# ghazalehnt/RecBole

Measured on AMD Instinct MI355X. Metric: train positives/sec (+neg) per node, higher is better.
Workload: dtype fp32; 1 GPU; C2 BPR-MF ml-20m-shape: 138,494 users x 26,745 items (incl. PAD), ~20M interactions RO_RS 0.8/0.1/0.1, embedding 128, 4 uniform negatives, 512 positives (2,048 rows) per step, dense Adam; global_batch=512, per_gpu_batch=512, train_interactions=16014928, parallelism=single, exchange_graph=True, sampler=walk (bit-exact)

## Files before the change

recbole_amd/csrc/adam.hip:

```cpp

#include "adam_core.h"

namespace mirec {

template <int D>
__global__ __launch_bounds__(kAdamThreads) void adam_multi_kernel(
    const AdamTables tabs, const float* __restrict__ consts, const int32_t* __restrict__ step_base,
    int step_off, AdamConsts k) {
  constexpr int VPR = D / 4;
  constexpr int RPP = kAdamThreads / VPR;
  static_assert(kAdamThreads % VPR == 0, "row width");
  __shared__ int32_t slot[kAdamRows];
  __shared__ int32_t s_range[2];

  const int si = segment_of(tabs, blockIdx.x);
  const mirec_adam_table& T = tabs.t[si];
  float* __restrict__ P = T.p;
  float* __restrict__ M = T.m;
  float* __restrict__ V = T.v;
  const int32_t* __restrict__ uniq = T.uniq;

  const int64_t lo = ((int64_t)blockIdx.x - tabs.block_start[si]) * kAdamRows;
  const int64_t hi = min(T.n_rows, lo + kAdamRows);
  if (threadIdx.x < kAdamRows) slot[threadIdx.x] = -1;
// ... 125 lines not shown
    const int i = base + rsub;
    const bool work = i < n;
    const int64_t r = lo + (work ? s_row[i] : 0);
    const int last = work ? min(s_last[i], target) : target;
    const int64_t off = r * VPR + c;
    V p, m, v;
    memset(&p, 0, sizeof(V));
    m = p;
    v = p;
    if (work) {
      p = reinterpret_cast<const V*>(T.p)[off];
      m = reinterpret_cast<const V*>(T.m)[off];
      v = reinterpret_cast<const V*>(T.v)[off];
    }
    adam_replay(p, m, v, last, target, consts, k);
    if (work) {
      reinterpret_cast<V*>(T.p)[off] = p;
      reinterpret_cast<V*>(T.m)[off] = m;
      reinterpret_cast<V*>(T.v)[off] = v;
      if (c == 0) T.last[r] = target;
    }
  }
}

template <int D>
struct FlushVec { using T = float; };
template <> struct FlushVec<128> { using T = float2; };
template <> struct FlushVec<256> { using T = float4; };

#ifndef MIREC_FLUSH_THREADS
#define MIREC_FLUSH_THREADS 64
#endif
constexpr int kFlushRowThreads = MIREC_FLUSH_THREADS;

template <int D>
__device__ __forceinline__ void flush_row(const mirec_adam_table& T, int64_t r, int raw,
                                          int target, int lane,
                                          const float* __restrict__ consts,
                                          const AdamConsts& k) {
  using V = typename FlushVec<D>::T;
  const int last = min(raw, target);
  const int64_t off = r * 64 + lane;
  const bool par = T.p_alt != nullptr;
  const bool odd = par && (target & 1);
  if (last >= target) {
    if (odd && raw != kZeroState)
      reinterpret_cast<V*>(T.p)[off] = reinterpret_cast<const V*>(T.p_alt)[off];
    return;
  }
  V p = reinterpret_cast<const V*>((par && (last & 1)) ? T.p_alt : T.p)[off];
  V m = reinterpret_cast<const V*>(T.m)[off];
  V v = reinterpret_cast<const V*>(T.v)[off];
  replay<V, true>(p, m, v, last, target, consts, k);
  MIREC_WORK(10, 1);
  if (odd) reinterpret_cast<V*>(T.p_alt)[off] = p;
  reinterpret_cast<V*>(T.p)[off] = p;
  reinterpret_cast<V*>(T.m)[off] = m;
  reinterpret_cast<V*>(T.v)[off] = v;
  if (lane == 0) T.last[r] = target;
}

__device__ __forceinline__ bool flush_needs(const mirec_adam_table& T, int raw, int target) {
  return min(raw, target) < target || (T.p_alt != nullptr && (target & 1) && raw != kZeroState);
}

template <int D>
__global__ __launch_bounds__(kFlushRowThreads) void adam_flush_row_kernel(
    const AdamTables tabs, const float* __restrict__ consts, const int32_t* __restrict__ step_base,
    int step_off, AdamConsts k) {
  constexpr int RPB = kFlushRowThreads / 64;
  const int si = segment_of(tabs, blockIdx.x);
  const mirec_adam_table& T = tabs.t[si];
  const int64_t r = ((int64_t)blockIdx.x - tabs.block_start[si]) * RPB + (threadIdx.x >> 6);
  if (r >= T.n_rows) return;
  const int target = step_base[0] + step_off;
  const int raw = __builtin_amdgcn_readfirstlane(T.last[r]);
  flush_row<D>(T, r, raw, target, threadIdx.x & 63, consts, k);
}

constexpr int64_t kScanOneWaveMax = 1 << 17;
struct FlushRows {
  int32_t r[kMaxTables];
};
struct FlushMasks {
  const uint32_t* bits[kMaxTables];
  int32_t want[kMaxTables];
};

__device__ __forceinline__ bool mask_selects(const uint32_t* __restrict__ bits, int want,
                                             int64_t r) {
  return !bits || (int)((bits[r >> 5] >> (r & 31)) & 1u) == want;
}

template <int D, bool MASKED>
__global__ __launch_bounds__(kAdamThreads) void adam_flush_scan_kernel(
    const AdamTables tabs, const float* __restrict__ consts, const int32_t* __restrict__ step_base,
    int step_off, AdamConsts k, FlushRows rows_per_wave, FlushMasks masks) {
  const int si = segment_of(tabs, blockIdx.x);
  const mirec_adam_table& T = tabs.t[si];
  const int R = rows_per_wave.r[si];
  const int lane = threadIdx.x & 63;
  const int64_t r0 =
      (((int64_t)blockIdx.x - tabs.block_start[si]) * (blockDim.x >> 6) + (threadIdx.x >> 6)) * R;
  if (r0 >= T.n_rows) return;
  const int target = step_base[0] + step_off;
  int raw = kZeroState;
  if (lane < R && r0 + lane < T.n_rows &&
      (!MASKED || mask_selects(masks.bits[si], masks.want[si], r0 + lane)))
    raw = T.last[r0 + lane];
  uint64_t todo = __ballot(flush_needs(T, raw, target));
  while (todo) {
    const int i = __builtin_ctzll(todo);
    todo &= todo - 1;
    flush_row<D>(T, r0 + i, __shfl(raw, i, 64), target, lane, consts, k);
  }
}

struct FlushFirst {
  const int32_t* first[kMaxTables];
};
constexpr int kFirstNotRead = MIREC_FIRST_NOT_READ;

template <int D>
__global__ __launch_bounds__(kAdamThreads) void adam_flush_first_kernel(
    const AdamTables tabs, const float* __restrict__ consts, const int32_t* __restrict__ step_base,
    int step_off, AdamConsts k, FlushRows rows_per_wave, FlushFirst ff) {
  const int si = segment_of(tabs, blockIdx.x);
  const mirec_adam_table& T = tabs.t[si];
  const int R = rows_per_wave.r[si];
  const int lane = threadIdx.x & 63;
  const int64_t r0 =
      (((int64_t)blockIdx.x - tabs.block_start[si]) * (blockDim.x >> 6) + (threadIdx.x >> 6)) * R;
  if (r0 >= T.n_rows) return;
  const int base = step_base[0] + step_off;
  int raw = kZeroState, target = 0;
  if (lane < R && r0 + lane < T.n_rows) {
    const int f = ff.first[si][r0 + lane];
    if (f > kFirstNotRead) {
      target = base + f;
      raw = T.last[r0 + lane];
    }
  }
  uint64_t todo = __ballot(min(raw, target) < target);
  while (todo) {
    const int i = __builtin_ctzll(todo);
    todo &= todo - 1;
    flush_row<D>(T, r0 + i, __builtin_amdgcn_readfirstlane(__shfl(raw, i, 64)),
                 __builtin_amdgcn_readfirstlane(__shfl(target, i, 64)), lane, consts, k);
  }
}

constexpr int kWalkRows = 32;

template <int D>
__global__ __launch_bounds__(64) void adam_flush_walk_kernel(
    const AdamTables tabs, const float* __restrict__ consts, const int32_t* __restrict__ step_base,
    int step_off, AdamConsts k, FlushMasks masks) {
  const int lane = threadIdx.x;
  const int target = step_base[0] + step_off;
  for (int si = 0; si < tabs.n_seg; ++si) {
    const mirec_adam_table& T = tabs.t[si];
    const uint32_t* __restrict__ bits = masks.bits[si];
    const uint32_t flip = masks.want[si] ? 0u : ~0u;
    const int64_t groups = (T.n_rows + kWalkRows - 1) / kWalkRows;
    for (int64_t g = blockIdx.x; g < groups; g += gridDim.x) {
      const int64_t r0 = g * kWalkRows;
      const uint32_t sel = bits ? (bits[g] ^ flip) : ~0u;
      int raw = kZeroState;
      if (lane < kWalkRows && r0 + lane < T.n_rows && ((sel >> lane) & 1u))
        raw = T.last[r0 + lane];
      uint64_t todo = __ballot(flush_needs(T, raw, target));
      while (todo) {
        const int i = __builtin_ctzll(todo);
        todo &= todo - 1;
        flush_row<D>(T, r0 + i, __shfl(raw, i, 64), target, lane, consts, k);
      }
    }
  }
}

}

using namespace mirec;

namespace {

enum class Sched { kStreamed, kDeferred, kFlush, kDeferredPair };

int launch_adam(Sched sched, const mirec_adam_table* tables, int32_t n_tables,
                const int64_t* n_max_uniq, int32_t d, const float* consts,
                const int32_t* step_base, int32_t step_off, double beta1, double beta2,
                double eps, double weight_decay, void* stream, const char* what,
                const int32_t* flush_rows = nullptr, const FlushMasks* masks = nullptr,
                int walk_waves = 0, const FlushFirst* firsts = nullptr) {
  if (n_tables < 1 || n_tables > kMaxTables || !tables || !consts || !step_base) {
    set_error("%s: bad arguments (n_tables=%d)", what, n_tables);
    return -1;
  }
  if (((uintptr_t)consts & 15) != 0) {
    set_error("%s: step constants must be 16-byte aligned", what);
    return -1;
  }
  if (d != 4 && d != 16 && d != 32 && d != 64 && d != 128 && d != 256 &&
      !(d == 1 && sched != Sched::kStreamed)) {
    set_error("%s: row width %d not in {4,16,32,64,128,256} (1: deferred / flush)", what, d);
    return -1;
  }
  const int VPR = d / 4;
  const bool pair = sched == Sched::kDeferredPair;
  if (pair) {
    if (n_tables != 2 || d == 1) {
      set_error("%s: a pair is two tables, the first of width d > 1 (got %d tables, d=%d)",
                what, n_tables, d);
      return -1;
    }
    sched = Sched::kDeferred;
  }
  FlushRows fr;
  bool scan = false;
  for (int q = 0; q < kMaxTables; ++q) fr.r[q] = 1;
  if (sched == Sched::kFlush && flush_rows) {
    if (d < 64) {
      set_error("%s: rows per wave need d >= 64", what);
      return -1;
    }
    for (int q = 0; q < n_tables; ++q) {
      if (flush_rows[q] < 1 || flush_rows[q] > 64) {
        set_error("%s: rows per wave %d of table %d not in [1, 64]", what, flush_rows[q], q);
        return -1;
      }
      fr.r[q] = flush_rows[q];
    }
    scan = true;
  }
  const bool walk = masks && walk_waves > 0;
  if (masks && (sched != Sched::kFlush || d < 64 || (!scan && !walk))) {
    set_error("%s: a masked flush needs d >= 64 and rows per wave or a wave count", what);
    return -1;
  }
  FlushMasks fm;
  memset(&fm, 0, sizeof(fm));
  if (masks) fm = *masks;
  if (firsts && (sched != Sched::kFlush || !scan || masks)) {
    set_error("%s: per-row targets need the flush with rows per wave and no mask", what);
    return -1;
  }
  FlushFirst ff;
  memset(&ff, 0, sizeof(ff));
  if (firsts) ff = *firsts;
  int scan_threads = kAdamThreads;
  if (scan && !walk) {
    int64_t waves = 0;
    for (int q = 0; q < n_tables; ++q)
      if (tables[q].n_rows > 0) waves += (tables[q].n_rows + fr.r[q] - 1) / fr.r[q];
    if (waves <= kScanOneWaveMax) scan_threads = 64;
  }
  AdamTables tabs;
  memset(&tabs, 0, sizeof(tabs));
  const bool deferred = sched == Sched::kDeferred;
  tabs.n_seg = deferred ? 2 * n_tables : n_tables;
  int dvec = 1;
  if (deferred && n_max_uniq && d >= 4) {
    int64_t waves = 0;
    for (int q = 0; q < (pair ? 1 : n_tables); ++q)
      if (n_max_uniq[q] > 0)
        waves += n_max_uniq[q] * (tables[q].ahead_uniq ? 2 : 1) * ((d + 63) / 64);
    if (waves > 16 * 1024) dvec = 2;
    bool ahead = false;
    for (int q = 0; q < n_tables; ++q) ahead = ahead || tables[q].ahead_uniq != nullptr;
    if (dvec == 2 && d >= 128 && !ahead && !pair) dvec = 4;
  }
  int64_t blocks = 0;
  for (int q = 0; q < n_tables; ++q) {
    const mirec_adam_table& t = tables[q];
    const bool grouped = t.n_uniq != nullptr;
    if (!t.p || !t.m || !t.v || t.n_rows < 0 ||
        (grouped && (!t.uniq || !t.seg || !t.perm || !t.rows)) ||
        (sched != Sched::kStreamed && !t.last) ||
        (deferred && (!grouped || t.dense_grad || !n_max_uniq || n_max_uniq[q] < 0)) ||
        (deferred && (t.ahead_uniq == nullptr) != (t.ahead_n_uniq == nullptr))) {
      set_error("%s: bad table %d", what, q);
      return -1;
    }
    if (t.p_alt && (sched == Sched::kStreamed || d < 64 || pair)) {
      set_error("%s: table %d: parity buffer (p_alt) needs the deferred schedule and d >= 64",
                what, q);
      return -1;
    }
    tabs.t[q] = t;
    if (walk) {
      tabs.block_start[q] = 0;
      if (t.n_rows > 0) blocks = walk_waves;
    } else if (deferred) {
      const int rpb = (pair && q == 1) ? deferred_block(1) : deferred_block(d / dvec) / (d / dvec);
      const int64_t nb = (n_max_uniq[q] + rpb - 1) / rpb;
      tabs.block_start[2 * q] = blocks;
      blocks += nb;
      tabs.block_start[2 * q + 1] = blocks;
      if (t.ahead_uniq) blocks += nb;
    } else {
      tabs.block_start[q] = blocks;
      const int64_t rows_per_block =
          scan ? (int64_t)(scan_threads / 64) * fr.r[q]
          : (sched == Sched::kFlush && d >= 64) ? kFlushRowThreads / 64
          : sched == Sched::kFlush ? kFlushRows
                                   : kAdamRows;
      blocks += (t.n_rows + rows_per_block - 1) / rows_per_block;
    }
  }
  (void)VPR;
  for (int q = tabs.n_seg; q <= 2 * kMaxTables; ++q) tabs.block_start[q] = blocks;
  if (blocks == 0) return 0;
  AdamConsts k;
  k.omb1 = (float)(1.0 - beta1);
  k.omb1m1 = k.omb1 - 1.0f;
  k.lerp_small = fabsf(k.omb1) < 0.5f;
  k.b2 = (float)beta2;
  k.omb2 = (float)(1.0 - beta2);
  k.eps = (float)eps;
  k.wd = (float)weight_decay;
  const dim3 grd((unsigned)blocks), blk(kAdamThreads);
  hipStream_t st = (hipStream_t)stream;
#define MIREC_ADAM_SCHED(DD)                                                                 \
  case DD:                                                                                   \
    if (sched == Sched::kStreamed)                                                           \
      hipLaunchKernelGGL(adam_multi_kernel<DD>, grd, blk, 0, st, tabs, consts, step_base,    \
                         step_off, k);                                                       \
    else if (deferred && pair)                                                               \
      hipLaunchKernelGGL((dvec == 2 ? adam_deferred_pair_kernel<DD, float2>                  \
                                    : adam_deferred_pair_kernel<DD, float>),                 \
                         grd, dim3(deferred_block(1)), 0, st, tabs, consts, step_base,       \
                         step_off, k);                                                       \
    else if (deferred)                                                                       \
      hipLaunchKernelGGL((dvec == 4 ? adam_deferred_kernel<DD, float4>                       \
                          : dvec == 2 ? adam_deferred_kernel<DD, float2>                     \
                                      : adam_deferred_kernel<DD, float>),                    \
                         grd, dim3(deferred_block(DD / dvec)), 0, st, tabs, consts,          \
                         step_base, step_off, k);                                            \
    else if (DD >= 64 && walk)                                                               \
      hipLaunchKernelGGL(adam_flush_walk_kernel<(DD >= 64 ? DD : 64)>, grd, dim3(64), 0, st,   \
                         tabs, consts, step_base, step_off, k, fm);                          \
    else if (DD >= 64 && scan && firsts)                                                     \
      hipLaunchKernelGGL(adam_flush_first_kernel<(DD >= 64 ? DD : 64)>, grd,                 \
                         dim3(scan_threads), 0, st, tabs, consts, step_base, step_off, k,    \
                         fr, ff);                                                            \
    else if (DD >= 64 && scan && masks)                                                      \
      hipLaunchKernelGGL((adam_flush_scan_kernel<(DD >= 64 ? DD : 64), true>), grd,          \
                         dim3(scan_threads), 0, st, tabs, consts, step_base, step_off, k,    \
                         fr, fm);                                                            \
    else if (DD >= 64 && scan)                                                               \
      hipLaunchKernelGGL((adam_flush_scan_kernel<(DD >= 64 ? DD : 64), false>), grd,         \
                         dim3(scan_threads), 0, st, tabs, consts, step_base, step_off, k,    \
                         fr, fm);                                                            \
    else if (DD >= 64)                                                                       \
      hipLaunchKernelGGL(adam_flush_row_kernel<(DD >= 64 ? DD : 64)>, grd,                   \
                         dim3(kFlushRowThreads), 0, st, tabs,                                \
                         consts, step_base, step_off, k);                                    \
    else                                                                                     \
      hipLaunchKernelGGL(adam_flush_list_kernel<(DD < 64 ? DD : 16)>, grd, blk, 0, st, tabs, \
                         consts, step_base, step_off, k);                                    \
    break;
  switch (d) {
    case 1:
      if (deferred)
        hipLaunchKernelGGL((adam_deferred_kernel<1, float>), grd, dim3(deferred_block(1)), 0, st,
                           tabs, consts, step_base, step_off, k);
      else
        hipLaunchKernelGGL(adam_flush_list_kernel<1>, grd, blk, 0, st, tabs, consts, step_base,
                           step_off, k);
      break;
    MIREC_ADAM_SCHED(4)
    MIREC_ADAM_SCHED(16)
    MIREC_ADAM_SCHED(32)
    MIREC_ADAM_SCHED(64)
    MIREC_ADAM_SCHED(128)
    MIREC_ADAM_SCHED(256)
  }
#undef MIREC_ADAM_SCHED
  return launch_status(what);
}

}

extern "C" int mirec_adam_multi_f32(const mirec_adam_table* tables, int32_t n_tables, int32_t d,
                                    const float* step_consts_dev, const int32_t* step_base_dev,
                                    int32_t step_off, double beta1, double beta2, double eps,
                                    double weight_decay, void* stream) {
  return launch_adam(Sched::kStreamed, tables, n_tables, nullptr, d, step_consts_dev,
                     step_base_dev, step_off, beta1, beta2, eps, weight_decay, stream,
                     "mirec_adam_multi_f32");
}

extern "C" int mirec_adam_deferred_f32(const mirec_adam_table* tables, int32_t n_tables,
                                       const int64_t* n_max_uniq, int32_t d,
                                       const float* step_consts_dev,
                                       const int32_t* step_base_dev, int32_t step_off,
                                       double beta1, double beta2, double eps,
                                       double weight_decay, void* stream) {
  return launch_adam(Sched::kDeferred, tables, n_tables, n_max_uniq, d, step_consts_dev,
                     step_base_dev, step_off, beta1, beta2, eps, weight_decay, stream,
                     "mirec_adam_deferred_f32");
}

extern "C" int mirec_adam_deferred_pair_f32(const mirec_adam_table* tables,
                                            const int64_t* n_max_uniq, int32_t d,
                                            const float* step_consts_dev,
                                            const int32_t* step_base_dev, int32_t step_off,
                                            double beta1, double beta2, double eps,
                                            double weight_decay, void* stream) {
  return launch_adam(Sched::kDeferredPair, tables, 2, n_max_uniq, d, step_consts_dev,
                     step_base_dev, step_off, beta1, beta2, eps, weight_decay, stream,
                     "mirec_adam_deferred_pair_f32");
}

extern "C" int mirec_adam_flush_f32(const mirec_adam_table* tables, int32_t n_tables, int32_t d,
                                    const float* step_consts_dev, const int32_t* step_base_dev,
                                    int32_t step_off, double beta1, double beta2, double eps,
                                    double weight_decay, void* stream) {
  return launch_adam(Sched::kFlush, tables, n_tables, nullptr, d, step_consts_dev,
                     step_base_dev, step_off, beta1, beta2, eps, weight_decay, stream,
                     "mirec_adam_flush_f32");
}

#if defined(MIREC_STEP_COUNT)
extern "C" int mirec_work_counters_adam(unsigned long long* dst, int clear) {
  if (hipMemcpyFromSymbol(dst, HIP_SYMBOL(g_work), sizeof(g_work)) != hipSuccess) return -1;
  if (clear) {
    unsigned long long z[16] = {0};
    if (hipMemcpyToSymbol(HIP_SYMBOL(g_work), z, sizeof(z)) != hipSuccess) return -1;
  }
  return 0;
}
#endif

extern "C" int mirec_adam_flush_rows_f32(const mirec_adam_table* tables, int32_t n_tables,
                                         int32_t d, const int32_t* rows_per_wave,
                                         const float* step_consts_dev,
                                         const int32_t* step_base_dev, int32_t step_off,
                                         double beta1, double beta2, double eps,
                                         double weight_decay, void* stream) {
  if (!rows_per_wave) {
    set_error("mirec_adam_flush_rows_f32: rows_per_wave is NULL");
    return -1;
  }
  return launch_adam(Sched::kFlush, tables, n_tables, nullptr, d, step_consts_dev,
                     step_base_dev, step_off, beta1, beta2, eps, weight_decay, stream,
                     "mirec_adam_flush_rows_f32", rows_per_wave);
}

extern "C" int mirec_adam_flush_masked_f32(const mirec_adam_table* tables, int32_t n_tables,
                                           int32_t d, const uint32_t* const* masks,
                                           const int32_t* want, const int32_t* rows_per_wave,
                                           int32_t walk_waves, const float* step_consts_dev,
                                           const int32_t* step_base_dev, int32_t step_off,
                                           double beta1, double beta2, double eps,
                                           double weight_decay, void* stream) {
  const char* what = "mirec_adam_flush_masked_f32";
  if (!tables || n_tables < 1 || n_tables > kMaxTables || !want || walk_waves < 0 ||
      walk_waves > 65536 || (walk_waves == 0) != (rows_per_wave != nullptr)) {
    set_error("%s: bad arguments (rows per wave for the scan form, or a wave count in "
              "[1, 65536] for the walk form)", what);
    return -1;
  }
  mirec_adam_table sel[kMaxTables];
  int32_t rows[kMaxTables];
  FlushMasks fm;
  memset(&fm, 0, sizeof(fm));
  int n = 0;
  for (int q = 0; q < n_tables; ++q) {
    if (want[q] < 0) continue;
    if (want[q] > 1) {
      set_error("%s: want[%d] = %d not in {-1, 0, 1}", what, q, want[q]);
      return -1;
    }
    sel[n] = tables[q];
    rows[n] = rows_per_wave ? rows_per_wave[q] : 1;
    fm.bits[n] = masks ? masks[q] : nullptr;
    fm.want[n] = want[q];
    ++n;
  }
  if (n == 0) return 0;
  return launch_adam(Sched::kFlush, sel, n, nullptr, d, step_consts_dev, step_base_dev, step_off,
                     beta1, beta2, eps, weight_decay, stream, what,
                     rows_per_wave ? rows : nullptr, &fm, walk_waves);
}

extern "C" int mirec_adam_flush_first_f32(const mirec_adam_table* tables, int32_t n_tables,
                                          int32_t d, const int32_t* const* first,
                                          const int32_t* rows_per_wave,
                                          const float* step_consts_dev,
                                          const int32_t* step_base_dev, int32_t step_off,
                                          double beta1, double beta2, double eps,
                                          double weight_decay, void* stream) {
  const char* what = "mirec_adam_flush_first_f32";
// ... 188 lines not shown
```

recbole_amd/csrc/step.hip:

```cpp
#include "adam_core.h"
#include "bpr_math.h"
#include "ahead.h"

namespace mirec {

struct StepLaunch {
  mirec_adam_table t[2];
  const int32_t* rec[2];
  const int32_t* crec[2];
  float* part[2];
  int32_t* join[2];
  int64_t block_start[7];
  int32_t seg_rows[6];
};

__device__ __forceinline__ int64_t clamp_id(int64_t id, int64_t n) {
  return id < 0 ? 0 : (id >= n ? n - 1 : id);
}


constexpr int kRecInts = 8;
constexpr int kRecInline = 2;
constexpr int kRowRec = 4 + kRecInline * kRecInts;
constexpr int kShare = kRecInline;
// ... 219 lines not shown
      run += c[j];
    }
  }
  __syncthreads();
#pragma unroll
  for (int r = 0; r < kGrpEpt; ++r) {
    const int e = tid + r * kGrpThreads;
    if (e < per) L.xb[L.bstart[keys[e] >> shift] + slot_in[r]] = x[r];
  }
  __syncthreads();
#pragma unroll
  for (int r = 0; r < kGrpEpt; ++r) {
    const int e = tid + r * kGrpThreads;
    if (e < per) {
      const int bk = keys[e] >> shift;
      const int b0 = L.bstart[bk], n = L.hist[bk];
      int rank = 0;
      for (int f = 0; f < n; ++f) rank += L.xb[b0 + f] < x[r] ? 1 : 0;
      L.xa[b0 + rank] = x[r];
    }
  }
  __syncthreads();
  const uint32_t* S = L.xa;
  int32_t* __restrict__ perm = J.perm + (int64_t)b * per;
  int32_t* __restrict__ uniq = J.uniq + (int64_t)b * per;
  int32_t* __restrict__ seg = J.seg + (int64_t)b * (per + 1);
  int hm = 0, cnt = 0;
#pragma unroll
  for (int r = 0; r < kGrpEpt; ++r) {
    const int e = kGrpEpt * tid + r;
    if (e < per) {
      const uint32_t k = S[e] >> pbits;
      const int h = (e == 0 || (S[e - 1] >> pbits) != k) ? 1 : 0;
      hm |= h << r;
      cnt += h;
      perm[e] = (int32_t)(S[e] & ((1u << pbits) - 1u));
    }
  }
  int nu;
  int slot = block_exclusive_scan(cnt, L.scan, &nu);
#pragma unroll
  for (int r = 0; r < kGrpEpt; ++r) {
    if ((hm >> r) & 1) {
      const int e = kGrpEpt * tid + r;
      const int32_t k = (int32_t)(S[e] >> pbits);
      L.srow[slot] = k;
      L.sseg[slot] = e;
      uniq[slot] = k;
      seg[slot] = e;
      ++slot;
    }
  }
  if (tid == 0) {
    L.sseg[nu] = per;
    seg[nu] = per;
    J.nu[b] = nu;
  }
  __syncthreads();
  if (J.rec != nullptr) {
    int32_t* __restrict__ rec = J.rec + (int64_t)b * rec_ints(per);
    int32_t* __restrict__ task = rec + (int64_t)per * kRowRec;
    const uint32_t pm = (1u << pbits) - 1u;
    int dealt = 0;
    for (int x0 = 0; x0 < nu; x0 += kGrpThreads) {
      const int xs = x0 + tid;
      int i0 = 0, nc = 0, row = 0;
      if (xs < nu) {
        i0 = L.sseg[xs];
        nc = L.sseg[xs + 1] - i0;
        row = L.srow[xs];
      }
      const int want = nc > kShare ? (nc + kShare - 1) / kShare - 1 : 0;
      int total;
      const int base = dealt + block_exclusive_scan(want, L.scan, &total);
      dealt += total;
      if (xs >= nu) continue;
      const int got = max(0, min(want, kSplitCap - base));
      const int nsh = 1 + got;
      int32_t* r = rec + (int64_t)xs * kRowRec;
      reinterpret_cast<int4*>(r)[0] = make_int4(row, i0, nc, nsh);
      for (int c = 0; c < kRecInline && c < nc; ++c)
        contrib_record_lds((int)(S[i0 + c] & pm), tb, Bc, T, L.uk, L.ik, r + 4 + c * kRecInts);
      for (int jj = 1; jj <= got; ++jj) {
        int32_t* tr = task + (int64_t)(base + jj - 1) * kTaskRec;
        reinterpret_cast<int4*>(tr)[0] = make_int4(xs, jj, i0, nc);
        reinterpret_cast<int4*>(tr)[1] = make_int4(row, nsh, 0, 0);
        for (int c = 0; c < kShare && jj * kShare + c < nc; ++c)
          contrib_record_lds((int)(S[i0 + jj * kShare + c] & pm), tb, Bc, T, L.uk, L.ik,
                             tr + 8 + c * kRecInts);
      }
    }
    if (tid == 0) task[(int64_t)kSplitCap * kTaskRec] = min(dealt, kSplitCap);
    int32_t* __restrict__ crec = J.crec + (int64_t)b * per * kRecInts;
    for (int e = tid; e < per; e += kGrpThreads)
      contrib_record_lds((int)(S[e] & pm), tb, Bc, T, L.uk, L.ik, crec + (int64_t)e * kRecInts);
  }
  if (ahead) {
    int32_t* __restrict__ out = J.ahead + (int64_t)(b - 1) * per;
    int base = 0;
    for (int x0 = 0; x0 < nu; x0 += kGrpThreads) {
      const int xs = x0 + tid;
      int f = 0;
      int32_t k = 0;
      if (xs < nu) {
        k = L.srow[xs];
        f = ((L.bits[k >> 5] >> (k & 31)) & 1u) ? 0 : 1;
      }
      int tot;
      const int ex = block_exclusive_scan(f, L.scan, &tot);
      if (f) out[base + ex] = k;
      base += tot;
    }
    if (tid == 0) J.nah[b - 1] = base;
  }
}

__device__ __forceinline__ void part_store(float* p, float4 a) {
  auto q = (__attribute__((address_space(1))) unsigned long long*)(p);
  const unsigned long long lo =
      (unsigned long long)__float_as_uint(a.x) | ((unsigned long long)__float_as_uint(a.y) << 32);
  const unsigned long long hi =
      (unsigned long long)__float_as_uint(a.z) | ((unsigned long long)__float_as_uint(a.w) << 32);
  __hip_atomic_store(q, lo, __ATOMIC_RELAXED, __HIP_MEMORY_SCOPE_AGENT);
  __hip_atomic_store(q + 1, hi, __ATOMIC_RELAXED, __HIP_MEMORY_SCOPE_AGENT);
}
__device__ __forceinline__ void part_load(const float* p, float& a) {
  auto q = (const __attribute__((address_space(1))) unsigned int*)(p);
  a = __uint_as_float(__hip_atomic_load(q, __ATOMIC_RELAXED, __HIP_MEMORY_SCOPE_AGENT));
}
__device__ __forceinline__ void part_load(const float* p, float2& a) {
  auto q = (const __attribute__((address_space(1))) unsigned long long*)(p);
  const unsigned long long w = __hip_atomic_load(q, __ATOMIC_RELAXED, __HIP_MEMORY_SCOPE_AGENT);
  a = make_float2(__uint_as_float((unsigned)w), __uint_as_float((unsigned)(w >> 32)));
}

constexpr int kJoinOrder = __ATOMIC_RELAXED;

template <typename V>
__device__ __forceinline__ void state_store(V* p, const V& x) {
  *p = x;
}

template <int D> struct StepVec { using T = float2; };
template <> struct StepVec<64> { using T = float; };
#ifndef MIREC_STEP_RPB
#define MIREC_STEP_RPB 4
#endif
template <int D> struct StepRows { static constexpr int n = D <= 128 ? MIREC_STEP_RPB : 1; };
#ifndef MIREC_STEP_SUM_LOADS
#define MIREC_STEP_SUM_LOADS 8
#endif
constexpr int kSumLoads = MIREC_STEP_SUM_LOADS;
#ifndef MIREC_STEP_WAVES
#define MIREC_STEP_WAVES 5
#endif
#ifndef MIREC_STEP_PRIO
#define MIREC_STEP_PRIO 3
#endif

template <int D>
__global__ __launch_bounds__(D / Lanes<typename StepVec<D>::T>::n * StepRows<D>::n,
                             MIREC_STEP_WAVES)
void bpr_adam_step_kernel(
    const StepLaunch L, const int64_t* __restrict__ items, int Bc, int T, float gamma,
    float grad_scale, float* __restrict__ loss_k, const float* __restrict__ consts,
    const int32_t* __restrict__ step_base, int step_off, AdamConsts k) {
  using V = typename StepVec<D>::T;
  constexpr int EPT = Lanes<V>::n;
  constexpr int TPB = D / EPT;
  constexpr int RPB = StepRows<D>::n;
  static_assert(RPB == 1 || TPB == 64, "several rows per workgroup need one wave per row");
  constexpr int LPR = D / 4;
  constexpr int NG = TPB / LPR;
  __builtin_amdgcn_s_setprio(MIREC_STEP_PRIO);
  __shared__ float cont_all[RPB][NG][D];
  __shared__ int s_last_all[RPB];
  const int wv = RPB > 1 ? __builtin_amdgcn_readfirstlane((int)(threadIdx.x / TPB)) : 0;
  auto& cont = cont_all[wv];
  int& s_last = s_last_all[wv];
  auto row_sync = [&]() {
    if (RPB == 1) {
      __syncthreads();
    } else {
      __builtin_amdgcn_fence(__ATOMIC_RELEASE, "wavefront");
      __builtin_amdgcn_wave_barrier();
      __builtin_amdgcn_fence(__ATOMIC_ACQUIRE, "wavefront");
    }
  };
  int si = 0;
#pragma unroll
  for (int q = 1; q < 6; ++q)
    if ((int64_t)blockIdx.x >= L.block_start[q]) si = q;
  const int kind = si >> 1;
  const bool ahead = kind == 1;
  const int tb = si & 1;
  const mirec_adam_table& T_ = L.t[tb];
  const int u = (int)(((int64_t)blockIdx.x - L.block_start[si]) * RPB) + wv;
  if (u >= L.seg_rows[si]) return;
  const int t = threadIdx.x - wv * TPB;
  const int grp = t / LPR;
  const int l = t - grp * LPR;
  const int per = tb ? (1 + T) * Bc : Bc;
  const int32_t* __restrict__ R = L.rec[tb];
  int4 h0 = make_int4(0, 0, 0, 0), h1 = h0, ra = h0, rb = h0;
  int n;
  int64_t row;
  if (ahead) {
    n = T_.ahead_n_uniq[0];
    row = T_.ahead_uniq[u];
  } else {
    const int32_t* __restrict__ Q;
    if (kind == 2) {
      n = T_.n_uniq[0];
      Q = R + (int64_t)u * kRowRec;
      h0 = reinterpret_cast<const int4*>(Q)[0];
      row = h0.x;
      Q += 4;
    } else {
      const int32_t* __restrict__ task = R + (int64_t)per * kRowRec;
      n = task[(int64_t)kSplitCap * kTaskRec];
      Q = task + (int64_t)u * kTaskRec;
      h0 = reinterpret_cast<const int4*>(Q)[0];
      h1 = reinterpret_cast<const int4*>(Q)[1];
      row = h1.x;
      Q += 8;
    }
    if (grp < kRecInline) {
      ra = reinterpret_cast<const int4*>(Q + grp * kRecInts)[0];
      rb = reinterpret_cast<const int4*>(Q + grp * kRecInts)[1];
    }
  }
  const int st = step_base[0] + step_off;
  if (u >= n) return;
  const float* __restrict__ Pr[2] = {T_.p, T_.p_alt};
  float* __restrict__ Pw = ((st + 1) & 1) ? T_.p_alt : T_.p;
  const int raw = T_.last[row];
  const int64_t off = row * (D / EPT) + t;

  if (ahead) {
    if (raw == kZeroState || raw > st) return;
    V p = reinterpret_cast<const V*>(Pr[raw & 1])[off];
    V m = reinterpret_cast<const V*>(T_.m)[off];
    V v = reinterpret_cast<const V*>(T_.v)[off];
    replay<V, true, 4>(p, m, v, raw, st, consts, k);
    V z;
    memset(&z, 0, sizeof(V));
    adam_vec(p, m, v, z, step_consts(consts, st), k);
    MIREC_WORK(3, EPT * MIREC_WORK_LANES());
    MIREC_WORK(5, 1);
    state_store(reinterpret_cast<V*>(Pw) + off, p);
    state_store(reinterpret_cast<V*>(T_.m) + off, m);
    state_store(reinterpret_cast<V*>(T_.v) + off, v);
    row_sync();
    if (t == 0) T_.last[row] = st + 1;
    return;
  }

  const int last = raw == kZeroState ? st : raw;
  V p = reinterpret_cast<const V*>(Pr[st & 1])[off];
  V m = reinterpret_cast<const V*>(T_.m)[off];
  V v = reinterpret_cast<const V*>(T_.v)[off];
  const float* __restrict__ EU = L.t[0].p;
  const float* __restrict__ EI = L.t[1].p;
  if (st & 1) {
    EU = L.t[0].p_alt;
    EI = L.t[1].p_alt;
  }
  const int x = kind == 2 ? u : h0.x;
  const int j = kind == 2 ? 0 : h0.y;
  const int i0 = kind == 2 ? h0.y : h0.z;
  const int nc = kind == 2 ? h0.z : h0.w;
  const int nsh = kind == 2 ? h0.w : h1.y;
  const bool split = nsh > 1;
  const int cnt = j ? min(kShare, nc - j * kShare)
                    : min(kShare, nc) + max(0, nc - nsh * kShare);
  const int cskip = (nsh - 1) * kShare;
  const float ng = -grad_scale;
  float* __restrict__ part = L.part[tb] + (int64_t)i0 * D;
  V g;
  memset(&g, 0, sizeof(V));
  __shared__ int4 xrec_all[RPB][kStepExtraCap][2];
  auto& xrec = xrec_all[wv];
  if (cnt > kRecInline) {
    const int32_t* __restrict__ C = L.crec[tb] + (int64_t)(i0 + cskip) * kRecInts;
    for (int c = kRecInline + t; c < min(cnt, kRecInline + kStepExtraCap); c += TPB) {
      xrec[c - kRecInline][0] = reinterpret_cast<const int4*>(C + (int64_t)c * kRecInts)[0];
      xrec[c - kRecInline][1] = reinterpret_cast<const int4*>(C + (int64_t)c * kRecInts)[1];
    }
    row_sync();
  }
  for (int base = 0; base < cnt; base += NG) {
    const int i = base + grp;
    if (i < cnt) {
      int4 r0 = ra, r1 = rb;
      if (i >= kRecInline) {
        if (i - kRecInline < kStepExtraCap) {
          r0 = xrec[i - kRecInline][0];
          r1 = xrec[i - kRecInline][1];
        } else {
          const int32_t* C = L.crec[tb] + (int64_t)(i0 + cskip + i) * kRecInts;
          r0 = reinterpret_cast<const int4*>(C)[0];
          r1 = reinterpret_cast<const int4*>(C)[1];
        }
      }
      const int kk = r0.x, jn = r0.y;
      if (l == 0) {
        if (jn >= 0) { MIREC_WORK(8, 1); } else if (tb == 0) { MIREC_WORK(6, 1); } else { MIREC_WORK(7, 1); }
      }
      const float4 uv = reinterpret_cast<const float4*>(EU + (int64_t)r0.z * D)[l];
      const float4 pv = reinterpret_cast<const float4*>(EI + (int64_t)r0.w * D)[l];
      float4 acc = make_float4(0.f, 0.f, 0.f, 0.f);
      if (jn >= 0) {
        const float4 nv = reinterpret_cast<const float4*>(EI + (int64_t)r1.x * D)[l];
        const float sp = group_sum<LPR>(dot4(uv, pv));
        const float sn = group_sum<LPR>(dot4(uv, nv));
        acc = contrib_n(bpr_coef(sp, sn, gamma, ng).dx, uv);
      } else {
        const int nid4[4] = {r1.x, r1.y, r1.z, r1.w};
        float lsum = 0.f;
        for (int j0 = 0; j0 < T; j0 += 4) {
          float4 nv[4];
#pragma unroll
          for (int e = 0; e < 4; ++e) {
            const int jj = j0 + e;
            nv[e] = make_float4(0.f, 0.f, 0.f, 0.f);
            if (jj < T) {
              const int64_t nid = jj < 4 ? (int64_t)nid4[e]
                                         : clamp_id(items[Bc + (int64_t)jj * Bc + kk],
                                                    L.t[1].n_rows);
              nv[e] = reinterpret_cast<const float4*>(EI + nid * D)[l];
            }
          }
          const float sp = group_sum<LPR>(dot4(uv, pv));
#pragma unroll
          for (int e = 0; e < 4; ++e) {
            const int jj = j0 + e;
            if (jj < T) {
              const float sn = group_sum<LPR>(dot4(uv, nv[e]));
              const BprCoef cf = bpr_coef(sp, sn, gamma, ng);
              lsum += cf.nll;
              if (tb == 0)
                contrib_u(acc, cf.dx, pv, nv[e]);
              else
                contrib_p(acc, cf.dx, uv);
            }
          }
        }
        if (tb == 0 && l == 0 && loss_k) loss_k[kk] = lsum;
      }
      if (split) {
        const int c = i < kShare ? j * kShare + i : cskip + i;
        part_store(part + (int64_t)c * D + 4 * l, acc);
      } else {
        *reinterpret_cast<float4*>(&cont[grp][4 * l]) = acc;
      }
    }
    if (!split) {
      row_sync();
#pragma unroll
      for (int h = 0; h < NG; ++h)
        if (base + h < cnt) {
          const V cv = *reinterpret_cast<const V*>(&cont[h][EPT * t]);
#pragma unroll
          for (int e = 0; e < EPT; ++e) Lanes<V>::at(g, e) += Lanes<V>::at(cv, e);
        }
      row_sync();
    }
  }
  if (split) MIREC_WORK(9, 1);
  if (split) {
    asm volatile("s_waitcnt vmcnt(0)" ::: "memory");
    row_sync();
    if (t == 0) {
      const int arrived =
          __hip_atomic_fetch_add(L.join[tb] + x, 1, kJoinOrder, __HIP_MEMORY_SCOPE_AGENT);
      s_last = arrived == nsh - 1;
      if (s_last) {
        __hip_atomic_store(L.join[tb] + x, 0, __ATOMIC_RELAXED, __HIP_MEMORY_SCOPE_AGENT);
        __builtin_amdgcn_fence(__ATOMIC_ACQUIRE, "agent");
        asm volatile("s_waitcnt vmcnt(0)" ::: "memory");
      }
    }
    row_sync();
    if (!s_last) return;
    const float* __restrict__ pe = part + EPT * t;
    int c = 0;
    for (; c + kSumLoads <= nc; c += kSumLoads) {
      V cv[kSumLoads];
#pragma unroll
      for (int h = 0; h < kSumLoads; ++h) part_load(pe + (int64_t)(c + h) * D, cv[h]);
#pragma unroll
      for (int h = 0; h < kSumLoads; ++h)
#pragma unroll
        for (int e = 0; e < EPT; ++e) Lanes<V>::at(g, e) += Lanes<V>::at(cv[h], e);
    }
    for (; c < nc; ++c) {
      V cv;
      part_load(pe + (int64_t)c * D, cv);
#pragma unroll
      for (int e = 0; e < EPT; ++e) Lanes<V>::at(g, e) += Lanes<V>::at(cv, e);
    }
  }
  if (last < st) {
    p = reinterpret_cast<const V*>(Pr[last & 1])[off];
  }

  replay<V, true>(p, m, v, last, st, consts, k);
  const bool fresh = last <= st;
  if (fresh) adam_vec(p, m, v, g, step_consts(consts, st), k);
  if (fresh) {
    MIREC_WORK(2, EPT * MIREC_WORK_LANES());
    MIREC_WORK(4, 1);
  }
  row_sync();
  if (!fresh) return;
  state_store(reinterpret_cast<V*>(Pw) + off, p);
  state_store(reinterpret_cast<V*>(T_.m) + off, m);
  state_store(reinterpret_cast<V*>(T_.v) + off, v);
  if (t == 0) T_.last[row] = st + 1;
}

}

using namespace mirec;

extern "C" int mirec_step_records(const int64_t* user_keys, const int64_t* item_keys,
                                  int64_t n_batches, int64_t Bc, int32_t T, int64_t n_users,
                                  int64_t n_items, const int32_t* u_perm, const int32_t* u_uniq,
                                  const int32_t* u_seg, const int32_t* u_nu,
                                  const int32_t* i_perm, const int32_t* i_uniq,
                                  const int32_t* i_seg, const int32_t* i_nu, int32_t* u_rec,
                                  int32_t* u_crec, int32_t* i_rec, int32_t* i_crec,
                                  int32_t* u_ahead, int32_t* u_nah, int32_t* i_ahead,
                                  int32_t* i_nah, void* stream) {
  if (n_batches < 0 || n_batches > 32767 || Bc < 0 || T < 1 ||
      (int64_t)(1 + T) * Bc > INT32_MAX || n_users <= 0 || n_items <= 0 || !user_keys || !item_keys || !u_perm || !u_uniq || !u_seg || !u_nu ||
      !i_perm || !i_uniq || !i_seg || !i_nu || !u_rec || !u_crec || !i_rec || !i_crec ||
      !u_ahead != !u_nah || !u_ahead != !i_ahead || !i_ahead != !i_nah) {
    set_error("mirec_step_records: bad arguments");
    return -1;
  }
  if (n_batches == 0 || Bc == 0) return 0;
  const RecJob U = {u_perm, u_uniq, u_seg, u_nu, u_rec, u_crec, u_ahead, u_nah};
  const RecJob I = {i_perm, i_uniq, i_seg, i_nu, i_rec, i_crec, i_ahead, i_nah};
  const int64_t KI = (1 + T) * Bc;
  const int PC = (int)((KI + kPrepThreads - 1) / kPrepThreads);
  hipLaunchKernelGGL(step_prep_kernel, dim3((unsigned)(4 * n_batches + 2 * n_batches * PC)),
                     dim3(kPrepThreads), 0, (hipStream_t)stream, user_keys, item_keys,
                     (int)n_batches, (int)Bc, T, n_users, n_items, U, I, PC);
  return launch_status("mirec_step_records");
}

extern "C" int64_t mirec_step_record_ints(int64_t per) { return per < 0 ? -1 : rec_ints(per); }

namespace mirec {
__global__ __launch_bounds__(256) void row_bitmap_kernel(const int64_t* __restrict__ keys,
                                                         int64_t n_keys, int64_t n_rows,
                                                         uint32_t* __restrict__ bitmap) {
  const int64_t i = (int64_t)blockIdx.x * blockDim.x + threadIdx.x;
  if (i >= n_keys) return;
  const int64_t r = clamp_id(keys[i], n_rows);
  atomicOr(bitmap + (r >> 5), 1u << (r & 31));
}
}

extern "C" int mirec_row_bitmap(const int64_t* keys, int64_t n_keys, int64_t n_rows,
                                uint32_t* bitmap, void* stream) {
  const char* what = "mirec_row_bitmap";
  if (n_keys < 0 || n_rows <= 0 || !bitmap || (n_keys > 0 && !keys) ||
      n_keys > (int64_t)INT32_MAX * 256) {
    set_error("%s: bad arguments", what);
    return -1;
  }
  hipStream_t st = (hipStream_t)stream;
  const int rc = hip_status(hipMemsetAsync(bitmap, 0, (size_t)((n_rows + 31) / 32) * 4, st), what);
  if (rc) return rc;
  if (n_keys == 0) return 0;
  hipLaunchKernelGGL(row_bitmap_kernel, dim3((unsigned)((n_keys + 255) / 256)), dim3(256), 0, st,
                     keys, n_keys, n_rows, bitmap);
  return launch_status(what);
}

namespace mirec {
__global__ __launch_bounds__(256) void first_read_kernel(const int32_t* __restrict__ uniq,
                                                         const int32_t* __restrict__ n_uniq,
                                                         int64_t per, int64_t n_rows,
                                                         uint32_t* __restrict__ first) {
  const int c = blockIdx.y;
  const int64_t i = (int64_t)blockIdx.x * blockDim.x + threadIdx.x;
  if (i >= per || i >= n_uniq[c]) return;
  const int64_t r = uniq[(int64_t)c * per + i];
  if (r < 0 || r >= n_rows) return;
  atomicMin(first + r, (uint32_t)c);
}
}

extern "C" int mirec_first_read(const int32_t* uniq, const int32_t* n_uniq, int64_t n_batches,
                                int64_t per, int64_t n_rows, int32_t* first, void* stream) {
  const char* what = "mirec_first_read";
  if (n_batches < 0 || n_batches > 32767 || per < 0 || per > INT32_MAX || n_rows <= 0 ||
      !first || (n_batches > 0 && per > 0 && (!uniq || !n_uniq))) {
    set_error("%s: bad arguments", what);
    return -1;
  }
  hipStream_t st = (hipStream_t)stream;
  static_assert(MIREC_FIRST_NOT_READ == -1, "reset by bytes of 0xff");
  const int rc = hip_status(hipMemsetAsync(first, 0xff, (size_t)n_rows * 4, st), what);
  if (rc) return rc;
  if (n_batches == 0 || per == 0) return 0;
  hipLaunchKernelGGL(first_read_kernel, dim3((unsigned)((per + 255) / 256), (unsigned)n_batches),
                     dim3(256), 0, st, uniq, n_uniq, per, n_rows,
                     reinterpret_cast<uint32_t*>(first));
  return launch_status(what);
}

#if defined(MIREC_STEP_COUNT)
extern "C" int mirec_work_counters(unsigned long long* dst, int clear) {
  if (hipMemcpyFromSymbol(dst, HIP_SYMBOL(g_work), sizeof(g_work)) != hipSuccess) return -1;
  if (clear) {
    unsigned long long z[16] = {0};
    if (hipMemcpyToSymbol(HIP_SYMBOL(g_work), z, sizeof(z)) != hipSuccess) return -1;
  }
  return 0;
}
#endif

namespace mirec {
static int bits_for(int64_t n) {
  int b = 0;
  while (b < 40 && ((int64_t)1 << b) < n) ++b;
  return b;
}
}

namespace mirec {
static bool chunk_group_fits(int64_t Bc, int32_t T, int64_t n_users, int64_t n_items,
                             bool ahead) {
  if (Bc <= 0 || T < 1 || n_users <= 0 || n_items <= 0) return false;
  const int64_t KI = (int64_t)(1 + T) * Bc;
  const int pu = bits_for(Bc), pi = bits_for(KI);
  return !(Bc > kGrpUserMax || KI > kGrpMax || bits_for(n_users) + pu > 32 ||
           bits_for(n_items) + pi > 32 ||
           (ahead && (n_users > 32 * (int64_t)kGrpBitmapWords ||
                      n_items > 32 * (int64_t)kGrpBitmapWords)));
}
}

extern "C" int mirec_chunk_group_fits(int64_t Bc, int32_t T, int64_t n_users, int64_t n_items,
                                      int32_t ahead) {
  return chunk_group_fits(Bc, T, n_users, n_items, ahead != 0) ? 1 : 0;
}

extern "C" int mirec_chunk_group(const int64_t* user_keys, const int64_t* item_keys,
                                 int64_t n_batches, int64_t Bc, int32_t T, int64_t n_users,
                                 int64_t n_items, int32_t* u_perm, int32_t* u_uniq,
                                 int32_t* u_seg, int32_t* u_nu, int32_t* i_perm,
                                 int32_t* i_uniq, int32_t* i_seg, int32_t* i_nu,
                                 int32_t* u_rec, int32_t* u_crec, int32_t* i_rec,
                                 int32_t* i_crec, int32_t* u_ahead, int32_t* u_nah,
                                 int32_t* i_ahead, int32_t* i_nah, void* stream) {
  if (n_batches < 0 || n_batches > 32767 || Bc < 0 || T < 1 || n_users <= 0 || n_items <= 0 ||
      !user_keys || !item_keys || !u_perm || !u_uniq || !u_seg || !u_nu || !i_perm || !i_uniq ||
      !i_seg || !i_nu || !u_rec != !u_crec || !u_rec != !i_rec || !i_rec != !i_crec ||
      !u_ahead != !u_nah || !u_ahead != !i_ahead || !i_ahead != !i_nah) {
    set_error("mirec_chunk_group: bad arguments");
    return -1;
  }
  if (n_batches == 0 || Bc == 0) return 1;
  const int64_t KI = (int64_t)(1 + T) * Bc;
  const int pu = bits_for(Bc), pi = bits_for(KI);
  if (!chunk_group_fits(Bc, T, n_users, n_items, u_ahead != nullptr)) return 0;
// ... 92 lines not shown
```

Before: 27.73 million positives/s.

## Split walk flush into per-table launches and trim step kernel addressing

```diff
diff --git a/recbole_amd/csrc/adam.hip b/recbole_amd/csrc/adam.hip
--- a/recbole_amd/csrc/adam.hip
+++ b/recbole_amd/csrc/adam.hip
@@ -301,6 +301,7 @@
 
 constexpr int kWalkRows = 32;
 
+#if defined(MIREC_WALK_WIDE)
 template <int D>
 __global__ __launch_bounds__(64) void adam_flush_walk_kernel(
     const AdamTables tabs, const float* __restrict__ consts, const int32_t* __restrict__ step_base,
@@ -327,6 +328,48 @@
     }
   }
 }
+#else
+struct WalkTable {
+  float* p;
+  float* p_alt;
+  float* m;
+  float* v;
+  int32_t* last;
+  const uint32_t* bits;
+  int64_t n_rows;
+  uint32_t flip;
+};
+
+template <int D>
+__global__ __launch_bounds__(64) void adam_flush_walk_kernel(
+    const WalkTable W, const float* __restrict__ consts, const int32_t* __restrict__ step_base,
+    int step_off, AdamConsts k) {
+  const int lane = threadIdx.x;
+  const int target = __builtin_amdgcn_readfirstlane(step_base[0] + step_off);
+  mirec_adam_table T;
+  memset(&T, 0, sizeof(T));
+  T.p = W.p;
+  T.p_alt = W.p_alt;
+  T.m = W.m;
+  T.v = W.v;
+  T.last = W.last;
+  T.n_rows = W.n_rows;
+  const int64_t groups = (W.n_rows + kWalkRows - 1) / kWalkRows;
+  for (int64_t g = blockIdx.x; g < groups; g += gridDim.x) {
+    const int64_t r0 = g * kWalkRows;
+    const int left = (int)min((int64_t)kWalkRows, W.n_rows - r0);
+    const uint32_t sel = W.bits ? (W.bits[g] ^ W.flip) : ~0u;
+    int raw = kZeroState;
+    if (lane < left && ((sel >> lane) & 1u)) raw = (W.last + r0)[lane];
+    uint64_t todo = __ballot(flush_needs(T, raw, target));
+    while (todo) {
+      const int i = __builtin_ctzll(todo);
+      todo &= todo - 1;
+      flush_row<D>(T, r0 + i, __builtin_amdgcn_readlane(raw, i), target, lane, consts, k);
+    }
+  }
+}
+#endif
 
 }
 
@@ -335,6 +378,32 @@
 namespace {
 
 enum class Sched { kStreamed, kDeferred, kFlush, kDeferredPair };
+
+template <int D>
+void launch_walk(const AdamTables& tabs, const FlushMasks& fm, dim3 grd, hipStream_t st,
+                 const float* consts, const int32_t* step_base, int step_off,
+                 const AdamConsts& k) {
+#if defined(MIREC_WALK_WIDE)
+  hipLaunchKernelGGL(adam_flush_walk_kernel<D>, grd, dim3(64), 0, st, tabs, consts, step_base,
+                     step_off, k, fm);
+#else
+  for (int q = 0; q < tabs.n_seg; ++q) {
+    const mirec_adam_table& t = tabs.t[q];
+    if (t.n_rows <= 0) continue;
+    WalkTable w;
+    w.p = t.p;
+    w.p_alt = t.p_alt;
+    w.m = t.m;
+    w.v = t.v;
+    w.last = t.last;
+    w.bits = fm.bits[q];
+    w.n_rows = t.n_rows;
+    w.flip = fm.want[q] ? 0u : ~0u;
+    hipLaunchKernelGGL(adam_flush_walk_kernel<D>, grd, dim3(64), 0, st, w, consts, step_base,
+                       step_off, k);
+  }
+#endif
+}
 
 int launch_adam(Sched sched, const mirec_adam_table* tables, int32_t n_tables,
                 const int64_t* n_max_uniq, int32_t d, const float* consts,
@@ -487,8 +556,7 @@
                          grd, dim3(deferred_block(DD / dvec)), 0, st, tabs, consts,          \
                          step_base, step_off, k);                                            \
     else if (DD >= 64 && walk)                                                               \
-      hipLaunchKernelGGL(adam_flush_walk_kernel<(DD >= 64 ? DD : 64)>, grd, dim3(64), 0, st,   \
-                         tabs, consts, step_base, step_off, k, fm);                          \
+      launch_walk<(DD >= 64 ? DD : 64)>(tabs, fm, grd, st, consts, step_base, step_off, k);  \
     else if (DD >= 64 && scan && firsts)                                                     \
       hipLaunchKernelGGL(adam_flush_first_kernel<(DD >= 64 ? DD : 64)>, grd,                 \
                          dim3(scan_threads), 0, st, tabs, consts, step_base, step_off, k,    \
diff --git a/recbole_amd/csrc/step.hip b/recbole_amd/csrc/step.hip
--- a/recbole_amd/csrc/step.hip
+++ b/recbole_amd/csrc/step.hip
@@ -395,7 +395,7 @@
 #endif
 constexpr int kSumLoads = MIREC_STEP_SUM_LOADS;
 #ifndef MIREC_STEP_WAVES
-#define MIREC_STEP_WAVES 5
+#define MIREC_STEP_WAVES 6
 #endif
 #ifndef MIREC_STEP_PRIO
 #define MIREC_STEP_PRIO 3
@@ -478,31 +478,32 @@
   const float* __restrict__ Pr[2] = {T_.p, T_.p_alt};
   float* __restrict__ Pw = ((st + 1) & 1) ? T_.p_alt : T_.p;
   const int raw = T_.last[row];
-  const int64_t off = row * (D / EPT) + t;
+  const int64_t rbase = (int64_t)__builtin_amdgcn_readfirstlane((int)row) * (D / EPT);
+  const unsigned tc = (unsigned)t;
 
   if (ahead) {
     if (raw == kZeroState || raw > st) return;
-    V p = reinterpret_cast<const V*>(Pr[raw & 1])[off];
-    V m = reinterpret_cast<const V*>(T_.m)[off];
-    V v = reinterpret_cast<const V*>(T_.v)[off];
+    V p = (reinterpret_cast<const V*>(Pr[raw & 1]) + rbase)[tc];
+    V m = (reinterpret_cast<const V*>(T_.m) + rbase)[tc];
+    V v = (reinterpret_cast<const V*>(T_.v) + rbase)[tc];
     replay<V, true, 4>(p, m, v, raw, st, consts, k);
     V z;
     memset(&z, 0, sizeof(V));
     adam_vec(p, m, v, z, step_consts(consts, st), k);
     MIREC_WORK(3, EPT * MIREC_WORK_LANES());
     MIREC_WORK(5, 1);
-    state_store(reinterpret_cast<V*>(Pw) + off, p);
-    state_store(reinterpret_cast<V*>(T_.m) + off, m);
-    state_store(reinterpret_cast<V*>(T_.v) + off, v);
+    state_store(reinterpret_cast<V*>(Pw) + rbase + tc, p);
+    state_store(reinterpret_cast<V*>(T_.m) + rbase + tc, m);
+    state_store(reinterpret_cast<V*>(T_.v) + rbase + tc, v);
     row_sync();
     if (t == 0) T_.last[row] = st + 1;
     return;
   }
 
   const int last = raw == kZeroState ? st : raw;
-  V p = reinterpret_cast<const V*>(Pr[st & 1])[off];
-  V m = reinterpret_cast<const V*>(T_.m)[off];
-  V v = reinterpret_cast<const V*>(T_.v)[off];
+  V p = (reinterpret_cast<const V*>(Pr[st & 1]) + rbase)[tc];
+  V m = (reinterpret_cast<const V*>(T_.m) + rbase)[tc];
+  V v = (reinterpret_cast<const V*>(T_.v) + rbase)[tc];
   const float* __restrict__ EU = L.t[0].p;
   const float* __restrict__ EI = L.t[1].p;
   if (st & 1) {
@@ -535,17 +536,18 @@
   for (int base = 0; base < cnt; base += NG) {
     const int i = base + grp;
     if (i < cnt) {
-      int4 r0 = ra, r1 = rb;
+      static_assert(NG >= kRecInline, "an inline record is used in round 0 only");
       if (i >= kRecInline) {
         if (i - kRecInline < kStepExtraCap) {
-          r0 = xrec[i - kRecInline][0];
-          r1 = xrec[i - kRecInline][1];
+          ra = xrec[i - kRecInline][0];
+          rb = xrec[i - kRecInline][1];
         } else {
           const int32_t* C = L.crec[tb] + (int64_t)(i0 + cskip + i) * kRecInts;
-          r0 = reinterpret_cast<const int4*>(C)[0];
-          r1 = reinterpret_cast<const int4*>(C)[1];
+          ra = reinterpret_cast<const int4*>(C)[0];
+          rb = reinterpret_cast<const int4*>(C)[1];
         }
       }
+      const int4 r0 = ra, r1 = rb;
       const int kk = r0.x, jn = r0.y;
       if (l == 0) {
         if (jn >= 0) { MIREC_WORK(8, 1); } else if (tb == 0) { MIREC_WORK(6, 1); } else { MIREC_WORK(7, 1); }
@@ -645,7 +647,7 @@
     }
   }
   if (last < st) {
-    p = reinterpret_cast<const V*>(Pr[last & 1])[off];
+    p = (reinterpret_cast<const V*>(Pr[last & 1]) + rbase)[tc];
   }
 
   replay<V, true>(p, m, v, last, st, consts, k);
@@ -657,9 +659,9 @@
   }
   row_sync();
   if (!fresh) return;
-  state_store(reinterpret_cast<V*>(Pw) + off, p);
-  state_store(reinterpret_cast<V*>(T_.m) + off, m);
-  state_store(reinterpret_cast<V*>(T_.v) + off, v);
+  state_store(reinterpret_cast<V*>(Pw) + rbase + tc, p);
+  state_store(reinterpret_cast<V*>(T_.m) + rbase + tc, m);
+  state_store(reinterpret_cast<V*>(T_.v) + rbase + tc, v);
   if (t == 0) T_.last[row] = st + 1;
 }
 
```

Result: faster. 28.59 million positives/s, median of 6 (+3.1%).
